# jason2714/de-i2i-gan

Hardware: AMD Instinct MI355X
Metric: paired 256x256 images/sec (G+D train step) (higher is better)
Workload: dtype bf16

## Files before the change

### de-i2i-gan_amd/csrc/wgrad_halo.hip

```cpp
#include <hip/hip_runtime.h>
#include <stdint.h>
#include <algorithm>

#include "common.h"
#include "geom.h"
#include "launch.h"

namespace dei2i {

__device__ __attribute__((aligned(256))) unsigned char g_zero_page_hw[256];

typedef __attribute__((address_space(3))) void lds_void_hw;
typedef __attribute__((address_space(1))) const void gbl_void_hw;

DEI2I_D void glds16hw(const void* gptr, unsigned char* lds_wave_base) { glds16_asm(gptr, lds_wave_base); }

constexpr int HW_TH = 4, HW_TW = 32;
constexpr int HW_HH = HW_TH + 2, HW_HWD = HW_TW + 2;
constexpr int HW_HPIX = HW_HH * HW_HWD;
constexpr int HW_HGROUPS = 26;
constexpr int HW_HPAD = HW_HGROUPS * 8;

template <int ROWB> DEI2I_D int hw_swz(int row) {
  if constexpr (ROWB == 256) return (row & 3) << 6;
  else return ((row >> 1) & 1) << 6;
}

template <int N> DEI2I_D void hw_wait_vm() { asm volatile("s_waitcnt vmcnt(%0)" ::"n"(N) : "memory"); }

template <int BCO, int BCI, int NTG, bool PRO = false>
__global__ __launch_bounds__(512) void wgrad_halo_kernel(const GatherDesc g, const bf16_t* __restrict__ src,
                                                         const bf16_t* __restrict__ dy, const int co_rows, const int ldy,
                                                         float* __restrict__ slabs, const int nslices, const int tiles_per_split,
                                                         const long long slab_elems, const ConvPro pro) {
  extern __shared__ __attribute__((aligned(16))) unsigned char smem[];
  const int tid = threadIdx.x, lane = tid & 63;
  const int wave = __builtin_amdgcn_readfirstlane(tid >> 6);
  constexpr int NIB = BCI / 32, NCB = BCO / 32;
  constexpr int TPW = (9 + NTG - 1) / NTG;
  static_assert(NCB * NIB * NTG == 8, "8 waves");
  constexpr int ROWB_A = BCO * 2, ROWB_B = BCI * 2;
  constexpr int HW_A_BYTES = 128 * ROWB_A, HW_B_BYTES = HW_HPAD * ROWB_B, HW_STAGE = HW_A_BYTES + HW_B_BYTES;
  constexpr int RPI_A = 1024 / ROWB_A, SPR_A = ROWB_A / 16;
  constexpr int RPI_B = 1024 / ROWB_B, SPR_B = ROWB_B / 16;
  constexpr int NA = 128 / RPI_A / 8, NB = (HW_HPAD / RPI_B + 7) / 8;
  constexpr int GROUPS_B = HW_HPAD / RPI_B;
  const int tg = wave / (NCB * NIB);
  const int cb = (wave / NIB) % NCB, ib = wave % NIB;
  const int tap0 = NTG == 1 ? 0 : tg * TPW;

  const int combo = blockIdx.y, split = blockIdx.x;
  const int tile_c = combo / nslices, slice = combo - tile_c * nslices;
  const int c0 = tile_c * BCO, ci0 = slice * BCI;

  const int tiles_x = g.Wo / HW_TW, tiles_y = g.Ho / HW_TH;
  const int tiles_img = tiles_x * tiles_y;
  const int ntiles = g.N * tiles_img;
  const int tbeg = split * tiles_per_split;
  const int tend = min(ntiles, tbeg + tiles_per_split);
  const bf16_t* zero = reinterpret_cast<const bf16_t*>(g_zero_page_hw);

  struct TileAt { int img, y0, x0; };
  auto tile_at = [&](int t) {
    TileAt q;
    q.img = t / tiles_img;
    const int rem = t - q.img * tiles_img;
    const int ty = rem / tiles_x;
    q.y0 = ty * HW_TH;
    q.x0 = (rem - ty * tiles_x) * HW_TW;
    return q;
  };
  auto tile_next = [&](TileAt& q) {
    q.x0 += HW_TW;
    if (q.x0 >= g.Wo) {
      q.x0 = 0;
      q.y0 += HW_TH;
      if (q.y0 >= g.Ho) { q.y0 = 0; ++q.img; }
    }
  };
  int a_off[NA];
  int b_hyx[NB], b_c[NB];
#pragma unroll
  for (int j = 0; j < NA; ++j) {
    const int rgrp = (j * 8 + wave) * RPI_A;
    const int r = rgrp + lane / SPR_A;
    const int off = ((lane % SPR_A) * 16) ^ hw_swz<ROWB_A>(r);
    const int c = c0 + (off >> 1);
    a_off[j] = c < ldy ? ((r >> 5) * g.Wo + (r & 31)) * ldy + c : -1;
    asm volatile("" : "+v"(a_off[j]));
  }
#pragma unroll
  for (int j = 0; j < NB; ++j) {
    int grp = j * 8 + wave;
    if (grp >= GROUPS_B) grp -= GROUPS_B;
    const int hp = grp * RPI_B + lane / SPR_B;
    const int hy = hp / HW_HWD, hx = hp - hy * HW_HWD;
    b_hyx[j] = hp < HW_HPIX ? ((hy << 16) | hx) : -1;
    b_c[j] = ci0 + ((((lane % SPR_B) * 16) ^ hw_swz<ROWB_B>(hp)) >> 1);
    asm volatile("" : "+v"(b_hyx[j]), "+v"(b_c[j]));
  }
  const bool fast = !PRO && g.pad_mode == PAD_REFLECT && c0 + BCO <= ldy;
  if (fast) {
#pragma unroll
    for (int j = 0; j < NB; ++j) {
      if (b_hyx[j] < 0) b_hyx[j] = 0;
    }
  }
  const unsigned smem_lds = lds_addr_of(smem);
  struct FastBase { const bf16_t* a; const bf16_t* b; int vy0, vx0; };
  auto fast_base = [&](const TileAt& q) {
    FastBase f;
    f.a = dy + (long long)((q.img * g.Ho + q.y0) * g.Wo + q.x0) * ldy;
    f.b = src + (size_t)q.img * ((size_t)g.Hs * g.Ws * g.Cs);
    f.vy0 = q.y0 + g.by0;
    f.vx0 = q.x0 + g.bx0;
    return f;
  };
  auto issue_a_fast = [&](int stage, const FastBase& f, int j) {
    const int rgrp = (j * 8 + wave) * RPI_A;
    glds16_asm_s(f.a, (unsigned)a_off[j] * 2u, smem_lds + stage * HW_STAGE + rgrp * ROWB_A);
  };
  auto issue_b_fast = [&](int stage, const FastBase& f, int j) {
    int grp = j * 8 + wave;
    if (grp >= GROUPS_B) grp -= GROUPS_B;
    const int vy = f.vy0 + (b_hyx[j] >> 16), vx = f.vx0 + (b_hyx[j] & 0xffff);
    const int ay = max(vy, -vy), ax = max(vx, -vx);
    const int y = min(ay, 2 * g.Hl - 2 - ay), x = min(ax, 2 * g.Wl - 2 - ax);
    const unsigned voff = (unsigned)(((y >> g.up) * g.Ws + (x >> g.up)) * g.Cs + b_c[j]) * 2u;
    glds16_asm_s(f.b, voff, smem_lds + stage * HW_STAGE + HW_A_BYTES + grp * 1024);
  };
  auto issue_a = [&](int stage, const TileAt& q, int j) {
    unsigned char* sa = smem + stage * HW_STAGE;
    const int rgrp = (j * 8 + wave) * RPI_A;
    const long long base = (long long)((q.img * g.Ho + q.y0) * g.Wo + q.x0) * ldy;
    const bf16_t* p = a_off[j] >= 0 ? dy + base + a_off[j] : zero;
    glds16hw(p, sa + rgrp * ROWB_A);
  };
  auto issue_b = [&](int stage, const TileAt& q, int j) {
    unsigned char* sb = smem + stage * HW_STAGE + HW_A_BYTES;
    int grp = j * 8 + wave;
    if (grp >= GROUPS_B) grp -= GROUPS_B;
    const bf16_t* p = zero;
    if (b_hyx[j] >= 0) {
      const int y = bound_coord(q.y0 + g.by0 + (b_hyx[j] >> 16), g.Hl, g.pad_mode);
      const int x = bound_coord(q.x0 + g.bx0 + (b_hyx[j] & 0xffff), g.Wl, g.pad_mode);
      if ((y | x) >= 0) {
        if (PRO && pro.ring != nullptr && !(ring_interior(y, g.Hl) && ring_interior(x, g.Wl)))
          p = pro.ring + ((size_t)(q.img * pro.ring_pix + ring_index(y, x, g.Hl, g.Wl))) * g.Cs + b_c[j];
        else
          p = src + (unsigned)(((q.img * g.Hs + (y >> g.up)) * g.Ws + (x >> g.up)) * g.Cs + b_c[j]);
      }
    }
    glds16hw(p, sb + grp * 1024);
  };
  auto issue = [&](int stage, const TileAt& q) {
    if (fast) {
      const FastBase f = fast_base(q);
#pragma unroll
      for (int j = 0; j < NA; ++j) issue_a_fast(stage, f, j);
#pragma unroll
      for (int j = 0; j < NB; ++j) issue_b_fast(stage, f, j);
      return;
    }
#pragma unroll
    for (int j = 0; j < NA; ++j) issue_a(stage, q, j);
#pragma unroll
    for (int j = 0; j < NB; ++j) issue_b(stage, q, j);
  };
  float* const pcoef = reinterpret_cast<float*>(smem + 2 * HW_STAGE);
  auto transform = [&](int stage, int t) {
    unsigned char* sb = smem + stage * HW_STAGE + HW_A_BYTES;
    const int img = t / tiles_img;
    const int rem = t - img * tiles_img;
    const int ty = rem / tiles_x;
    const int y0 = ty * HW_TH, x0 = (rem - ty * tiles_x) * HW_TW;
    for (int v = tid; v < HW_HPIX * SPR_B; v += 512) {
      const int hp = v / SPR_B, sl = v - hp * SPR_B;
      const int hy = hp / HW_HWD, hx = hp - hy * HW_HWD;
      const int y = bound_coord(y0 + g.by0 + hy, g.Hl, g.pad_mode);
      const int x = bound_coord(x0 + g.bx0 + hx, g.Wl, g.pad_mode);
      if ((y | x) < 0) continue;
      if (pro.ring != nullptr && !(ring_interior(y, g.Hl) && ring_interior(x, g.Wl))) continue;
      const int cofs = ((sl * 16) ^ hw_swz<ROWB_B>(hp)) >> 1;
      float A8[8], B8[8], f[8];
      ldcoef<8>(pcoef + cofs, A8);
      ldcoef<8>(pcoef + BCI + cofs, B8);
      u32x4* p = reinterpret_cast<u32x4*>(sb + hp * ROWB_B + sl * 16);
      Elem<bf16_t>::unpack(*p, f);
#pragma unroll
      for (int e = 0; e < 8; ++e) {
        const float w = fmaf(A8[e], f[e], B8[e]);
        f[e] = fmaf(pro.slope, fminf(w, 0.f), fmaxf(w, 0.f));
      }
      *p = Elem<bf16_t>::pack(f);
    }
  };

  f32x16 acc[TPW];
#pragma unroll
  for (int t = 0; t < TPW; ++t)
#pragma unroll
    for (int e = 0; e < 16; ++e) acc[t][e] = 0.f;

  const int lr = lane & 31, lh = lane >> 5;
  const int tr_q = (lane & 15) >> 2, tr_p = lane & 3, tr_half = (lane >> 4) & 1;
  const int a_colb = (cb * 32 + 16 * tr_half + 4 * tr_p) * 2;
  const int b_colb = (ib * 32 + 16 * tr_half + 4 * tr_p) * 2;

  auto tr_read = [&](const unsigned char* base, int o0, int o1) {
    s16x4 lo = __builtin_amdgcn_ds_read_tr16_b64_v4i16((__attribute__((address_space(3))) s16x4*)(base + o0));
    s16x4 hi = __builtin_amdgcn_ds_read_tr16_b64_v4i16((__attribute__((address_space(3))) s16x4*)(base + o1));
    u32x2 l2 = __builtin_bit_cast(u32x2, lo), h2 = __builtin_bit_cast(u32x2, hi);
    u32x4 r;
    r.x = l2.x; r.y = l2.y; r.z = h2.x; r.w = h2.y;
    return r;
  };

  auto compute = [&](int stage) {
    const unsigned char* ab = smem + stage * HW_STAGE;
    const unsigned char* bb = ab + HW_A_BYTES;
#pragma unroll 2
    for (int kb = 0; kb < 8; ++kb) {
      const int ra = kb * 16 + 8 * lh + tr_q;
      const u32x4 af = tr_read(ab, ra * ROWB_A + (a_colb ^ hw_swz<ROWB_A>(ra)), (ra + 4) * ROWB_A + (a_colb ^ hw_swz<ROWB_A>(ra + 4)));
      const int py = kb >> 1, px0 = (kb & 1) * 16;
#pragma unroll
      for (int t = 0; t < TPW; ++t) {
        const int tap = tap0 + t;
        if (NTG > 1 && tap >= 9) break;
        const int ty = tap / 3, tx = tap - ty * 3;
        const int rb = (py + ty) * HW_HWD + px0 + tx + 8 * lh + tr_q;
        const u32x4 bf = tr_read(bb, rb * ROWB_B + (b_colb ^ hw_swz<ROWB_B>(rb)), (rb + 4) * ROWB_B + (b_colb ^ hw_swz<ROWB_B>(rb + 4)));
        acc[t] = __builtin_amdgcn_mfma_f32_32x32x16_bf16(__builtin_bit_cast(bf16x8, af), __builtin_bit_cast(bf16x8, bf), acc[t], 0, 0, 0);
      }
    }
  };

  const int nt = tend - tbeg;
  int cur_img = -1;
  TileAt nxt = tile_at(tbeg);
#pragma unroll 1
  for (int it = -1; it < nt; ++it) {
    if (it >= 0) {
      asm volatile("s_waitcnt vmcnt(0)" ::: "memory");
      __builtin_amdgcn_s_barrier();
    }
    bool reload = false;
    float cval = 0.f;
    if constexpr (PRO) {
      if (it >= 0 && pro.A != nullptr) {
        const int img = (tbeg + it) / tiles_img;
        reload = img != cur_img;
        if (reload && tid < 2 * BCI)
          cval = (tid < BCI ? pro.A : pro.B)[(size_t)img * pro.n_stride + ci0 + (tid < BCI ? tid : tid - BCI)];
        cur_img = img;
      }
    }
    if (it + 1 < nt) issue((it + 1) & 1, nxt);
    if constexpr (PRO) {
      if (it >= 0 && pro.A != nullptr) {
        if (reload) {
          if (it + 1 < nt) hw_wait_vm<NA + NB>(); else hw_wait_vm<0>();
          if (tid < 2 * BCI) pcoef[tid] = cval;
          __syncthreads();
        }
        transform(it & 1, tbeg + it);
        asm volatile("s_waitcnt lgkmcnt(0)" ::: "memory");
        __builtin_amdgcn_s_barrier();
      }
    }
    if (it >= 0) compute(it & 1);
    tile_next(nxt);
  }

  float* slab = slabs + (size_t)split * slab_elems;
  const int co_w = __builtin_amdgcn_readfirstlane(c0 + cb * 32);
  float* p0 = slab + (size_t)(co_w + 4 * lh) * g.K + ci0 + ib * 32 + lr;
#pragma unroll
  for (int t = 0; t < TPW; ++t) {
    const int tap = tap0 + t;
    if (NTG > 1 && tap >= 9) break;
    float* pt = p0 + tap * g.Cs;
#pragma unroll
    for (int q = 0; q < 4; ++q) {
      if (co_w + 8 * q >= co_rows) break;
#pragma unroll
      for (int r = 0; r < 4; ++r) pt[(size_t)(8 * q + r) * g.K] = acc[t][q * 4 + r];
    }
  }
}

template <int BCO, int BCI, int NTG>
static hipError_t launch_wgrad_halo(const GatherDesc& g, const void* src, const void* dy, int co_rows, int ldy, float* slabs,
                                    size_t slab_capacity_elems, int num_cu, int* nsplit_out, bool force, hipStream_t st,
                                    const ConvPro* pro) {
  const int nslices = g.Cs / BCI, tiles_c = (co_rows + BCO - 1) / BCO;
  const int combos = nslices * tiles_c;
  const int ntiles = g.N * (g.Ho / HW_TH) * (g.Wo / HW_TW);
  int splits = std::max(1, num_cu / combos);
  if (splits > 8) splits -= splits % 8;
  if (splits > ntiles / 4) splits = std::max(1, ntiles / 4);
  const long long slab_elems = wgrad_slab_elems(co_rows, g.K);
  if ((size_t)slab_elems * splits > slab_capacity_elems) splits = (int)(slab_capacity_elems / (size_t)slab_elems);
  if (splits < 1) return hipErrorNotSupported;
  if (!force && combos * splits < (num_cu * 3) / 4) return hipErrorNotSupported;
  const int tps = (ntiles + splits - 1) / splits;
  const int zs = (ntiles + tps - 1) / tps;
  const size_t lds = 2 * (size_t)(128 * BCO * 2 + HW_HPAD * BCI * 2) + (pro != nullptr ? 2 * BCI * sizeof(float) : 0);
  auto kern = pro != nullptr ? wgrad_halo_kernel<BCO, BCI, NTG, true> : wgrad_halo_kernel<BCO, BCI, NTG, false>;
  static bool attr_done[2] = {false, false};
  const int which = pro != nullptr ? 1 : 0;
  if (!attr_done[which]) {
    hipError_t e = hipFuncSetAttribute(reinterpret_cast<const void*>(kern), hipFuncAttributeMaxDynamicSharedMemorySize, (int)lds);
    if (e != hipSuccess) return e;
    attr_done[which] = true;
  }
  const ConvPro pv = pro != nullptr ? *pro : ConvPro{nullptr, nullptr, 0, 0.f, nullptr, 0};
  count_launch(K_WGRAD_HALO);
  prof_begin(PROF_WGRAD, 2.0 * (double)g.M * 9.0 * (double)g.Clog * (double)co_rows, st);
  hipLaunchKernelGGL(kern, dim3(zs, combos), dim3(512), lds, st, g, (const bf16_t*)src, (const bf16_t*)dy, co_rows, ldy, slabs,
                     nslices, tps, slab_elems, pv);
  prof_end(PROF_WGRAD, st);
  *nsplit_out = zs;
  return hipGetLastError();
}

hipError_t wgrad_halo(const GatherDesc& g, const void* src, const void* dy, int co_rows, int ldy, float* slabs,
                      size_t slab_capacity_elems, int num_cu, int* nsplit_out, bool force, hipStream_t st, const ConvPro* pro) {
  if (pro != nullptr && pro->ring != nullptr && (g.Hl < 4 || g.Wl < 4)) return hipErrorNotSupported;
  if (g.sh != 1 || g.sw != 1 || g.ys != 1 || g.xs != 1 || g.th != 3 || g.tw != 3) return hipErrorNotSupported;
  if (g.Ho % HW_TH != 0 || g.Wo % HW_TW != 0) return hipErrorNotSupported;
  if ((long long)g.N * g.Hs * g.Ws * g.Cs >= (1ll << 31)) return hipErrorNotSupported;
  if (co_rows <= 64) {
    if (g.Cs % 128 == 0 && co_rows >= 48)
      return launch_wgrad_halo<64, 128, 1>(g, src, dy, co_rows, ldy, slabs, slab_capacity_elems, num_cu, nsplit_out, force, st, pro);
    if (g.Cs % 64 == 0 && co_rows <= 32)
      return launch_wgrad_halo<64, 64, 2>(g, src, dy, co_rows, ldy, slabs, slab_capacity_elems, num_cu, nsplit_out, force, st, pro);
    return hipErrorNotSupported;
  }
  if (g.Cs % 64 != 0 || co_rows < 96) return hipErrorNotSupported;
  return launch_wgrad_halo<128, 64, 1>(g, src, dy, co_rows, ldy, slabs, slab_capacity_elems, num_cu, nsplit_out, force, st, pro);
}

}
```

Before: 467.5.

## Iterate halo rows in weight-grad kernel to reuse B fragments across taps

For the single-tap-group case, the 3x3 weight-gradient inner loop now walks halo rows instead of output k-blocks. Each B fragment is read from LDS once per halo row and half and reused across all vertical taps, and A fragments sit in a small rotating register buffer. LDS addresses are precomputed per lane with a 4-way swizzle table and pinned with empty asm to cut address arithmetic. This lowers LDS transpose-read traffic and ALU overhead, at the cost of more registers and full unrolling. The multi-tap-group path is unchanged.

```diff
diff --git a/de-i2i-gan_amd/csrc/wgrad_halo.hip b/de-i2i-gan_amd/csrc/wgrad_halo.hip
--- a/de-i2i-gan_amd/csrc/wgrad_halo.hip
+++ b/de-i2i-gan_amd/csrc/wgrad_halo.hip
@@ -216,23 +216,80 @@
     return r;
   };
 
+  typedef __attribute__((address_space(3))) s16x4* lds_s16x4_ptr;
+  auto tr_read_lds = [&](unsigned a0, unsigned a1) {
+    s16x4 lo = __builtin_amdgcn_ds_read_tr16_b64_v4i16((lds_s16x4_ptr)(uintptr_t)a0);
+    s16x4 hi = __builtin_amdgcn_ds_read_tr16_b64_v4i16((lds_s16x4_ptr)(uintptr_t)a1);
+    u32x2 l2 = __builtin_bit_cast(u32x2, lo), h2 = __builtin_bit_cast(u32x2, hi);
+    u32x4 r;
+    r.x = l2.x; r.y = l2.y; r.z = h2.x; r.w = h2.y;
+    return r;
+  };
+  const int lq = 8 * lh + tr_q;
+  const int a_lane = lq * ROWB_A + (a_colb ^ hw_swz<ROWB_A>(lq));
+  int b_lane[4];
+#pragma unroll
+  for (int k = 0; k < 4; ++k) b_lane[k] = lq * ROWB_B + (b_colb ^ hw_swz<ROWB_B>(k + lq));
+  auto compute_rows = [&](int stage) {
+    if constexpr (NTG == 1) {
+      unsigned ab = smem_lds + stage * HW_STAGE + a_lane;
+      unsigned bk[4];
+      asm volatile("" : "+v"(ab));
+#pragma unroll
+      for (int k = 0; k < 4; ++k) {
+        bk[k] = smem_lds + stage * HW_STAGE + HW_A_BYTES + b_lane[k];
+        asm volatile("" : "+v"(bk[k]));
+      }
+      u32x4 af[3][2];
+#pragma unroll
+      for (int hy = 0; hy < HW_HH; ++hy) {
+#pragma unroll
+        for (int half = 0; half < 2; ++half) {
+          if (hy < HW_TH) {
+            const int ra = (hy * 2 + half) * 16;
+            af[hy % 3][half] = tr_read_lds(ab + ra * ROWB_A, ab + (ra + 4) * ROWB_A);
+          }
+          u32x4 bf[3];
+#pragma unroll
+          for (int tx = 0; tx < 3; ++tx) {
+            const int rb = hy * HW_HWD + half * 16 + tx;
+            bf[tx] = tr_read_lds(bk[rb & 3] + rb * ROWB_B, bk[rb & 3] + (rb + 4) * ROWB_B);
+          }
+#pragma unroll
+          for (int ty = 0; ty < 3; ++ty) {
+            const int py = hy - ty;
+            if (py < 0 || py >= HW_TH) continue;
+#pragma unroll
+            for (int tx = 0; tx < 3; ++tx)
+              acc[3 * ty + tx] = __builtin_amdgcn_mfma_f32_32x32x16_bf16(__builtin_bit_cast(bf16x8, af[py % 3][half]),
+                                                                         __builtin_bit_cast(bf16x8, bf[tx]), acc[3 * ty + tx], 0, 0, 0);
+          }
+        }
+      }
+    }
+  };
+
   auto compute = [&](int stage) {
-    const unsigned char* ab = smem + stage * HW_STAGE;
-    const unsigned char* bb = ab + HW_A_BYTES;
+    if constexpr (NTG > 1) {
+      const unsigned char* ab = smem + stage * HW_STAGE;
+      const unsigned char* bb = ab + HW_A_BYTES;
 #pragma unroll 2
-    for (int kb = 0; kb < 8; ++kb) {
-      const int ra = kb * 16 + 8 * lh + tr_q;
-      const u32x4 af = tr_read(ab, ra * ROWB_A + (a_colb ^ hw_swz<ROWB_A>(ra)), (ra + 4) * ROWB_A + (a_colb ^ hw_swz<ROWB_A>(ra + 4)));
-      const int py = kb >> 1, px0 = (kb & 1) * 16;
-#pragma unroll
-      for (int t = 0; t < TPW; ++t) {
-        const int tap = tap0 + t;
-        if (NTG > 1 && tap >= 9) break;
-        const int ty = tap / 3, tx = tap - ty * 3;
-        const int rb = (py + ty) * HW_HWD + px0 + tx + 8 * lh + tr_q;
-        const u32x4 bf = tr_read(bb, rb * ROWB_B + (b_colb ^ hw_swz<ROWB_B>(rb)), (rb + 4) * ROWB_B + (b_colb ^ hw_swz<ROWB_B>(rb + 4)));
-        acc[t] = __builtin_amdgcn_mfma_f32_32x32x16_bf16(__builtin_bit_cast(bf16x8, af), __builtin_bit_cast(bf16x8, bf), acc[t], 0, 0, 0);
-      }
+      for (int kb = 0; kb < 8; ++kb) {
+        const int ra = kb * 16 + 8 * lh + tr_q;
+        const u32x4 af = tr_read(ab, ra * ROWB_A + (a_colb ^ hw_swz<ROWB_A>(ra)), (ra + 4) * ROWB_A + (a_colb ^ hw_swz<ROWB_A>(ra + 4)));
+        const int py = kb >> 1, px0 = (kb & 1) * 16;
+#pragma unroll
+        for (int t = 0; t < TPW; ++t) {
+          const int tap = tap0 + t;
+          if (tap >= 9) break;
+          const int ty = tap / 3, tx = tap - ty * 3;
+          const int rb = (py + ty) * HW_HWD + px0 + tx + 8 * lh + tr_q;
+          const u32x4 bf = tr_read(bb, rb * ROWB_B + (b_colb ^ hw_swz<ROWB_B>(rb)), (rb + 4) * ROWB_B + (b_colb ^ hw_swz<ROWB_B>(rb + 4)));
+          acc[t] = __builtin_amdgcn_mfma_f32_32x32x16_bf16(__builtin_bit_cast(bf16x8, af), __builtin_bit_cast(bf16x8, bf), acc[t], 0, 0, 0);
+        }
+      }
+    } else {
+      compute_rows(stage);
     }
   };
 
```

Result: faster. 473.8 (median of 6 runs) (+1.3%).
